# akuendig/cuda-matrix-inversion

Measured on AMD Instinct MI355X. Metric: matrix inversions/s, higher is better.
Workload: dtype f64; 1 GPU; gj64: 100000 x 64x64 fp64 Gauss-Jordan, SPD inputs (natural-order pivots verified inside the MFMA sweep; a rejected matrix is redone with partial pivoting), BASELINE configs[2]; n=64, total_batch=100000, batch_per_gpu=100000, algorithm=gj, kernel=matinv_gj_tile_f64<4, true, true>, input=SPD: R + R^T + n I

## Files before the change

### cuda-matrix-inversion_amd/csrc/tile_gj_kernels.hip

```cpp
#include "tile_impl.hpp"

namespace matinv {

template hipError_t launch_gj_tile<double>(int, BatchRef<const double>, BatchRef<double>, size_t, int *, hipStream_t);

}
```

### cuda-matrix-inversion_amd/csrc/tile_impl.hpp

```cpp
#pragma once
#include <stdio.h>
#include <stdlib.h>
#include <string.h>
#include <atomic>

#include "tile_common.hpp"
#include "tile_screen.hpp"

namespace matinv {


#define MATINV_PREP_ROW(MOV, b, a) MOV " %" #b ", %" #a "\n\t" MOV " %" #a ", 0\n\t"
#define MATINV_PREP_ZERO(MOV, a) MOV " %" #a ", 0\n\t"
#define MATINV_PREP_TAIL(MOV, save, eye) MOV " %0, %" #eye "\n\ts_nop 1\n\ts_mov_b64 exec, %" #save
#define MATINV_PREP_SAVE(save, mask) "s_and_saveexec_b64 %" #save ", %" #mask "\n\t"
template <int NT, class T>
__device__ __forceinline__ void prep_operands(typename TileGeo<T>::vec4 (&acc)[NT][NT], T (&bop)[NT], int kb, T eye)
{
    static_assert(NT >= 1 && NT <= 4, "prep_operands: one asm text per tile count");
    const int tK = kb >> 2, rK = kb & 3;
    const unsigned long long pmask = sizeof(T) == 8 ? 0x000F000F000F000FULL << (4 * rK) : 0x1111111111111111ULL << rK;
    unsigned long long save;
    auto J = [&](int i) { return (tK + i) % NT; };
    auto R = [&](int i) { return (rK + i) & 3; };
#define ROW(i) acc[tK][J(i)][rK]
#define COL(i, r) acc[J(i)][tK][R(r)]
    if constexpr (sizeof(T) == 8) {
#define MV "v_mov_b64_e32"
        if constexpr (NT == 1)
            asm volatile(MATINV_PREP_ROW(MV, 0, 1) MATINV_PREP_SAVE(5, 6)
                         MATINV_PREP_ZERO(MV, 2) MATINV_PREP_ZERO(MV, 3) MATINV_PREP_ZERO(MV, 4) MATINV_PREP_TAIL(MV, 5, 7)
                         : "=&v"(bop[J(0)]), "+v"(ROW(0)), "+v"(COL(0, 1)), "+v"(COL(0, 2)), "+v"(COL(0, 3)), "=&s"(save)
                         : "s"(pmask), "v"(eye) : "scc");
        else if constexpr (NT == 2)
            asm volatile(MATINV_PREP_ROW(MV, 0, 2) MATINV_PREP_ROW(MV, 1, 3) MATINV_PREP_SAVE(11, 12)
                         MATINV_PREP_ZERO(MV, 4) MATINV_PREP_ZERO(MV, 5) MATINV_PREP_ZERO(MV, 6)
                         MATINV_PREP_ZERO(MV, 7) MATINV_PREP_ZERO(MV, 8) MATINV_PREP_ZERO(MV, 9) MATINV_PREP_ZERO(MV, 10)
                         MATINV_PREP_TAIL(MV, 11, 13)
                         : "=&v"(bop[J(0)]), "=&v"(bop[J(1)]), "+v"(ROW(0)), "+v"(ROW(1)),
                           "+v"(COL(0, 1)), "+v"(COL(0, 2)), "+v"(COL(0, 3)),
                           "+v"(COL(1, 0)), "+v"(COL(1, 1)), "+v"(COL(1, 2)), "+v"(COL(1, 3)), "=&s"(save)
                         : "s"(pmask), "v"(eye) : "scc");
        else if constexpr (NT == 3)
            asm volatile(MATINV_PREP_ROW(MV, 0, 3) MATINV_PREP_ROW(MV, 1, 4) MATINV_PREP_ROW(MV, 2, 5) MATINV_PREP_SAVE(17, 18)
                         MATINV_PREP_ZERO(MV, 6) MATINV_PREP_ZERO(MV, 7) MATINV_PREP_ZERO(MV, 8)
                         MATINV_PREP_ZERO(MV, 9) MATINV_PREP_ZERO(MV, 10) MATINV_PREP_ZERO(MV, 11) MATINV_PREP_ZERO(MV, 12)
                         MATINV_PREP_ZERO(MV, 13) MATINV_PREP_ZERO(MV, 14) MATINV_PREP_ZERO(MV, 15) MATINV_PREP_ZERO(MV, 16)
                         MATINV_PREP_TAIL(MV, 17, 19)
                         : "=&v"(bop[J(0)]), "=&v"(bop[J(1)]), "=&v"(bop[J(2)]), "+v"(ROW(0)), "+v"(ROW(1)), "+v"(ROW(2)),
                           "+v"(COL(0, 1)), "+v"(COL(0, 2)), "+v"(COL(0, 3)),
                           "+v"(COL(1, 0)), "+v"(COL(1, 1)), "+v"(COL(1, 2)), "+v"(COL(1, 3)),
                           "+v"(COL(2, 0)), "+v"(COL(2, 1)), "+v"(COL(2, 2)), "+v"(COL(2, 3)), "=&s"(save)
                         : "s"(pmask), "v"(eye) : "scc");
        else
            asm volatile(MATINV_PREP_ROW(MV, 0, 4) MATINV_PREP_ROW(MV, 1, 5) MATINV_PREP_ROW(MV, 2, 6) MATINV_PREP_ROW(MV, 3, 7)
                         MATINV_PREP_SAVE(23, 24)
                         MATINV_PREP_ZERO(MV, 8) MATINV_PREP_ZERO(MV, 9) MATINV_PREP_ZERO(MV, 10)
                         MATINV_PREP_ZERO(MV, 11) MATINV_PREP_ZERO(MV, 12) MATINV_PREP_ZERO(MV, 13) MATINV_PREP_ZERO(MV, 14)
                         MATINV_PREP_ZERO(MV, 15) MATINV_PREP_ZERO(MV, 16) MATINV_PREP_ZERO(MV, 17) MATINV_PREP_ZERO(MV, 18)
                         MATINV_PREP_ZERO(MV, 19) MATINV_PREP_ZERO(MV, 20) MATINV_PREP_ZERO(MV, 21) MATINV_PREP_ZERO(MV, 22)
                         MATINV_PREP_TAIL(MV, 23, 25)
                         : "=&v"(bop[J(0)]), "=&v"(bop[J(1)]), "=&v"(bop[J(2)]), "=&v"(bop[J(3)]),
                           "+v"(ROW(0)), "+v"(ROW(1)), "+v"(ROW(2)), "+v"(ROW(3)),
                           "+v"(COL(0, 1)), "+v"(COL(0, 2)), "+v"(COL(0, 3)),
                           "+v"(COL(1, 0)), "+v"(COL(1, 1)), "+v"(COL(1, 2)), "+v"(COL(1, 3)),
                           "+v"(COL(2, 0)), "+v"(COL(2, 1)), "+v"(COL(2, 2)), "+v"(COL(2, 3)),
                           "+v"(COL(3, 0)), "+v"(COL(3, 1)), "+v"(COL(3, 2)), "+v"(COL(3, 3)), "=&s"(save)
                         : "s"(pmask), "v"(eye) : "scc");
#undef MV
    } else {
#define MV "v_mov_b32_e32"
        if constexpr (NT == 1)
            asm volatile(MATINV_PREP_ROW(MV, 0, 1) MATINV_PREP_SAVE(5, 6)
                         MATINV_PREP_ZERO(MV, 2) MATINV_PREP_ZERO(MV, 3) MATINV_PREP_ZERO(MV, 4) MATINV_PREP_TAIL(MV, 5, 7)
                         : "=&v"(bop[J(0)]), "+v"(ROW(0)), "+v"(COL(0, 1)), "+v"(COL(0, 2)), "+v"(COL(0, 3)), "=&s"(save)
                         : "s"(pmask), "v"(eye) : "scc");
        else if constexpr (NT == 2)
            asm volatile(MATINV_PREP_ROW(MV, 0, 2) MATINV_PREP_ROW(MV, 1, 3) MATINV_PREP_SAVE(11, 12)
                         MATINV_PREP_ZERO(MV, 4) MATINV_PREP_ZERO(MV, 5) MATINV_PREP_ZERO(MV, 6)
                         MATINV_PREP_ZERO(MV, 7) MATINV_PREP_ZERO(MV, 8) MATINV_PREP_ZERO(MV, 9) MATINV_PREP_ZERO(MV, 10)
                         MATINV_PREP_TAIL(MV, 11, 13)
                         : "=&v"(bop[J(0)]), "=&v"(bop[J(1)]), "+v"(ROW(0)), "+v"(ROW(1)),
                           "+v"(COL(0, 1)), "+v"(COL(0, 2)), "+v"(COL(0, 3)),
                           "+v"(COL(1, 0)), "+v"(COL(1, 1)), "+v"(COL(1, 2)), "+v"(COL(1, 3)), "=&s"(save)
                         : "s"(pmask), "v"(eye) : "scc");
        else if constexpr (NT == 3)
            asm volatile(MATINV_PREP_ROW(MV, 0, 3) MATINV_PREP_ROW(MV, 1, 4) MATINV_PREP_ROW(MV, 2, 5) MATINV_PREP_SAVE(17, 18)
                         MATINV_PREP_ZERO(MV, 6) MATINV_PREP_ZERO(MV, 7) MATINV_PREP_ZERO(MV, 8)
                         MATINV_PREP_ZERO(MV, 9) MATINV_PREP_ZERO(MV, 10) MATINV_PREP_ZERO(MV, 11) MATINV_PREP_ZERO(MV, 12)
                         MATINV_PREP_ZERO(MV, 13) MATINV_PREP_ZERO(MV, 14) MATINV_PREP_ZERO(MV, 15) MATINV_PREP_ZERO(MV, 16)
                         MATINV_PREP_TAIL(MV, 17, 19)
                         : "=&v"(bop[J(0)]), "=&v"(bop[J(1)]), "=&v"(bop[J(2)]), "+v"(ROW(0)), "+v"(ROW(1)), "+v"(ROW(2)),
                           "+v"(COL(0, 1)), "+v"(COL(0, 2)), "+v"(COL(0, 3)),
                           "+v"(COL(1, 0)), "+v"(COL(1, 1)), "+v"(COL(1, 2)), "+v"(COL(1, 3)),
                           "+v"(COL(2, 0)), "+v"(COL(2, 1)), "+v"(COL(2, 2)), "+v"(COL(2, 3)), "=&s"(save)
                         : "s"(pmask), "v"(eye) : "scc");
        else
            asm volatile(MATINV_PREP_ROW(MV, 0, 4) MATINV_PREP_ROW(MV, 1, 5) MATINV_PREP_ROW(MV, 2, 6) MATINV_PREP_ROW(MV, 3, 7)
                         MATINV_PREP_SAVE(23, 24)
                         MATINV_PREP_ZERO(MV, 8) MATINV_PREP_ZERO(MV, 9) MATINV_PREP_ZERO(MV, 10)
                         MATINV_PREP_ZERO(MV, 11) MATINV_PREP_ZERO(MV, 12) MATINV_PREP_ZERO(MV, 13) MATINV_PREP_ZERO(MV, 14)
                         MATINV_PREP_ZERO(MV, 15) MATINV_PREP_ZERO(MV, 16) MATINV_PREP_ZERO(MV, 17) MATINV_PREP_ZERO(MV, 18)
                         MATINV_PREP_ZERO(MV, 19) MATINV_PREP_ZERO(MV, 20) MATINV_PREP_ZERO(MV, 21) MATINV_PREP_ZERO(MV, 22)
                         MATINV_PREP_TAIL(MV, 23, 25)
                         : "=&v"(bop[J(0)]), "=&v"(bop[J(1)]), "=&v"(bop[J(2)]), "=&v"(bop[J(3)]),
                           "+v"(ROW(0)), "+v"(ROW(1)), "+v"(ROW(2)), "+v"(ROW(3)),
                           "+v"(COL(0, 1)), "+v"(COL(0, 2)), "+v"(COL(0, 3)),
                           "+v"(COL(1, 0)), "+v"(COL(1, 1)), "+v"(COL(1, 2)), "+v"(COL(1, 3)),
                           "+v"(COL(2, 0)), "+v"(COL(2, 1)), "+v"(COL(2, 2)), "+v"(COL(2, 3)),
                           "+v"(COL(3, 0)), "+v"(COL(3, 1)), "+v"(COL(3, 2)), "+v"(COL(3, 3)), "=&s"(save)
                         : "s"(pmask), "v"(eye) : "scc");
#undef MV
    }
#undef ROW
#undef COL
}
#undef MATINV_PREP_ROW
#undef MATINV_PREP_ZERO
#undef MATINV_PREP_TAIL
#undef MATINV_PREP_SAVE

template <class T, int NT, bool FULL, bool LOOKAHEAD, bool EARLY = false>
__device__ __forceinline__ void gj_tile_body(BatchRef<const T> Ain, BatchRef<T> Xout, int *info, int n_rt, unsigned batch,
                                             int *work_count, int *work_list, T *panel, const int *in_count, const int *in_list)
{
    typedef TileGeo<T> G;
    typedef typename G::vec4 vec4;
    typedef typename G::vec2 vec2;
    constexpr int N = 16 * NT;
    constexpr int NKB = 4 * NT;
    constexpr bool PAIRED = FULL && (NT % 2 == 0);
    const int l = threadIdx.x;

    const unsigned todo = in_count ? (unsigned)*in_count : batch;
    for (unsigned item = blockIdx.x; item < todo; item += gridDim.x) {
        const unsigned mat = in_list ? (unsigned)in_list[item] : item;
        const T *A = Ain.at_uniform(mat);
        T *X = Xout.at_uniform(mat);
        int n = FULL ? N : n_rt;
        if (!FULL) asm volatile("" : "+s"(n));
        int q = l >> 4, c = l & 15;
        const unsigned lane_off = (unsigned)(G::trow(0, l >> 4) * n + (l & 15));
        asm volatile("" : "+v"(q), "+v"(c));
        const T eye = G::piv(c) == q ? (T)1 : (T)0;
        vec4 acc[NT][NT];
        if (PAIRED) {
            const unsigned lane_off2 = (unsigned)(2 * G::trow(0, l >> 4) * N + 2 * (l & 15));
#pragma unroll
            for (int ti = 0; ti < NT; ++ti)
#pragma unroll
                for (int u = 0; u < NT / 2; ++u)
#pragma unroll
                    for (int r = 0; r < 4; ++r) {
                        const unsigned uoff = (unsigned)((32 * (ti >> 1) + 2 * G::trow(r, 0) + (ti & 1)) * N + 32 * u);
                        const vec2 v = __builtin_nontemporal_load(reinterpret_cast<const vec2 *>(A + uoff + lane_off2));
                        acc[ti][2 * u][r] = v[0];
                        acc[ti][2 * u + 1][r] = v[1];
                    }
        } else {
#pragma unroll
            for (int ti = 0; ti < NT; ++ti)
#pragma unroll
                for (int tj = 0; tj < NT; ++tj)
#pragma unroll
                    for (int r = 0; r < 4; ++r) {
                        const int row = 16 * ti + G::trow(r, q), col = 16 * tj + c;
                        const unsigned uoff = (unsigned)((16 * ti + G::trow(r, 0)) * n + 16 * tj);
                        const bool edge = !FULL && (ti == NT - 1 || tj == NT - 1);
                        acc[ti][tj][r] = (!edge || (row < n && col < n)) ? A[uoff + lane_off] : ((row == col) ? (T)1 : (T)0);
                    }
        }
        unsigned long long bad = 0;
        T aop[NT], bop[NT];

#ifdef MATINV_TILE_LDST_ONLY
        if (false) {
#else
        if (LOOKAHEAD) {
#endif
            panel_to_lds<NT, T>(panel, acc, 0, q, c);
            wave_lds_sync();
            panel_solve<NT>(panel, 0, q, c, aop, bad);
#pragma unroll
            for (int kb = 0; kb < NKB; ++kb) {
                if (!FULL && kb > 4 * (NT - 1) && kb - 4 * (NT - 1) >= G::real_blocks(n - 16 * (NT - 1))) continue;
                prep_operands<NT, T>(acc, bop, kb, eye);
                if (kb + 1 < NKB) {
                    const int tn = (kb + 1) >> 2;
#pragma unroll
                    for (int ti = 0; ti < NT; ++ti)
                        acc[ti][tn] = G::mfma(aop[ti], bop[tn], acc[ti][tn]);
                    constexpr int NB = NT * (NT - 1);
                    int pend = 0;
                    auto issue_b = [&](int count) {
#pragma unroll
                        for (int z = 0; z < count; ++z) {
                            if (pend < NB) {
                                const int tjx = pend / NT, ti = pend % NT;
                                const int tj = tjx + (tjx >= tn ? 1 : 0);
                                acc[ti][tj] = G::mfma(aop[ti], bop[tj], acc[ti][tj]);
                                ++pend;
                            }
                        }
                        __builtin_amdgcn_sched_barrier(0);
                    };
                    __builtin_amdgcn_sched_barrier(0);
                    issue_b(2);
                    wave_lds_sync();
                    panel_to_lds<NT, T>(panel, acc, kb + 1, q, c);
                    wave_lds_sync();
                    __builtin_amdgcn_sched_barrier(0);
                    T aop_next[NT];
                    PanelSolve<NT, false, T> ps;
                    constexpr int NS = PanelSolve<NT, false, T>::NSTAGE;
#pragma unroll
                    for (int s = 0; s < NS; ++s) {
                        issue_b(((NB - 2) * (s + 1)) / NS - ((NB - 2) * s) / NS);
                        ps.stage(s, panel, kb + 1, q, c, aop_next, bad);
                        __builtin_amdgcn_sched_barrier(0);
                    }
                    issue_b(NB);
#pragma unroll
                    for (int ti = 0; ti < NT; ++ti) aop[ti] = aop_next[ti];
                    if (EARLY && NT > 1 && kb == 3 && bad != 0) break;
                } else {
#pragma unroll
                    for (int ti = 0; ti < NT; ++ti)
#pragma unroll
                        for (int tj = 0; tj < NT; ++tj)
                            acc[ti][tj] = G::mfma(aop[ti], bop[tj], acc[ti][tj]);
                }
            }
        } else {
#ifdef MATINV_TILE_LDST_ONLY
            (void)aop, (void)bop;
#else
#pragma unroll
            for (int kb = 0; kb < NKB; ++kb) {
                if (!FULL && kb > 4 * (NT - 1) && kb - 4 * (NT - 1) >= G::real_blocks(n - 16 * (NT - 1))) continue;
                panel_to_lds<NT, T>(panel, acc, kb, q, c);
                wave_lds_sync();
                panel_solve<NT>(panel, kb, q, c, aop, bad);
                wave_lds_sync();
                prep_operands<NT, T>(acc, bop, kb, eye);
#pragma unroll
                for (int ti = 0; ti < NT; ++ti)
#pragma unroll
                    for (int tj = 0; tj < NT; ++tj)
                        acc[ti][tj] = G::mfma(aop[ti], bop[tj], acc[ti][tj]);
            }
#endif
        }

        if (bad == 0) {
            if (PAIRED) {
                const unsigned lane_off2 = (unsigned)(2 * G::trow(0, l >> 4) * N + 2 * (l & 15));
#pragma unroll
                for (int ti = 0; ti < NT; ++ti)
#pragma unroll
                    for (int u = 0; u < NT / 2; ++u)
#pragma unroll
                        for (int r = 0; r < 4; ++r) {
                            const unsigned uoff = (unsigned)((32 * (ti >> 1) + 2 * G::trow(r, 0) + (ti & 1)) * N + 32 * u);
                            vec2 v;
                            v[0] = acc[ti][2 * u][r];
                            v[1] = acc[ti][2 * u + 1][r];
                            __builtin_nontemporal_store(v, reinterpret_cast<vec2 *>(X + uoff + lane_off2));
                        }
            } else {
#pragma unroll
                for (int ti = 0; ti < NT; ++ti)
#pragma unroll
                    for (int tj = 0; tj < NT; ++tj)
#pragma unroll
                        for (int r = 0; r < 4; ++r) {
                            const int row = 16 * ti + G::trow(r, q), col = 16 * tj + c;
                            const unsigned uoff = (unsigned)((16 * ti + G::trow(r, 0)) * n + 16 * tj);
                            const bool edge = !FULL && (ti == NT - 1 || tj == NT - 1);
                            if (!edge || (row < n && col < n)) X[uoff + lane_off] = acc[ti][tj][r];
                        }
            }
            if (info && l == 0) info[mat] = 0;
        } else if (l == 0) {
            const int slot = atomicAdd(work_count, 1);
            work_list[slot] = (int)mat;
        }
        if (LOOKAHEAD) wave_lds_sync();
    }
}


template <int NT, bool FULL, bool LOOKAHEAD, bool EARLY = false>
__global__ __launch_bounds__(64, 2) void matinv_gj_tile_f64(BatchRef<const double> Ain,
                                                                                 BatchRef<double> Xout, int *info,
                                                                                 int n_rt, unsigned batch,
                                                                                 int *work_count, int *work_list, const int *in_count,
                                                                                 const int *in_list)
{
    __shared__ __attribute__((aligned(16))) double panel[16 * NT * 4];
    gj_tile_body<double, NT, FULL, LOOKAHEAD, EARLY>(Ain, Xout, info, n_rt, batch, work_count, work_list, panel, in_count, in_list);
}

template <int NT, bool FULL, bool LOOKAHEAD, bool EARLY = false>
__global__ __launch_bounds__(64, FULL ? 4 : 3) void matinv_gj_tile_f32(BatchRef<const float> Ain, BatchRef<float> Xout, int *info,
                                                           int n_rt, unsigned batch, int *work_count, int *work_list, const int *in_count,
                                                           const int *in_list)
{
    __shared__ __attribute__((aligned(16))) float panel[16 * NT * 4];
    gj_tile_body<float, NT, FULL, LOOKAHEAD, EARLY>(Ain, Xout, info, n_rt, batch, work_count, work_list, panel, in_count, in_list);
}

template <class T>
struct SpdGp {
    const T *a, *c, *d, *e;
    T *out;
};

template <class T, int NT, bool FULL, bool GP = false>
__device__ __forceinline__ void spd_tile_body(BatchRef<const T> Ain, BatchRef<T> Xout, int *info, int n_rt, unsigned batch,
                                              int *work_count, int *work_list, T *panel, SpdGp<T> gp = SpdGp<T>())
{
    typedef TileGeo<T> G;
    typedef typename G::vec4 vec4;
    constexpr int N = 16 * NT;
    constexpr int NKB = 4 * NT;
    constexpr int TSTRIDE = 17;
    const int l = threadIdx.x;

    for (unsigned mat = blockIdx.x; mat < batch; mat += gridDim.x) {
        const T *A = Ain.at_uniform(mat);
        T *X = Xout.at_uniform(mat);
        int n = FULL ? N : n_rt;
        if (!FULL) asm volatile("" : "+s"(n));
        int q = l >> 4, c = l & 15;
        const unsigned lane_off = (unsigned)((l >> 4) * n + (l & 15));
        asm volatile("" : "+v"(q), "+v"(c));

        vec4 acc[NT][NT];
#pragma unroll
        for (int ti = 0; ti < NT; ++ti)
#pragma unroll
            for (int tj = 0; tj < NT; ++tj) {
                if (tj > ti) continue;
#pragma unroll
                for (int r = 0; r < 4; ++r) {
                    const int row = 16 * ti + G::trow(r, q), col = 16 * tj + c;
                    T v;
                    if (ti == tj) {
                        const int hi = row > col ? row : col, lo = row > col ? col : row;
                        v = (FULL || ti < NT - 1 || (row < n && col < n)) ? A[(unsigned)(lo * n + hi)] : ((row == col) ? (T)1 : (T)0);
                        if (GP && row == col && (FULL || ti < NT - 1 || row < n)) v += gp.c[(size_t)mat * n + row];
                    } else {
                        v = (FULL || ti < NT - 1 || (row < n && col < n)) ? A[(unsigned)(col * n + row)] : (T)0;
                    }
                    acc[ti][tj][r] = v;
                }
            }
        (void)lane_off;
        unsigned long long bad = 0;
        T aop[NT], bop[NT];

        spd_panel_to_lds<NT, T>(panel, acc, 0, q, c);
        wave_lds_sync();
        {
            PanelSolve<NT, true, T> ps0;
#pragma unroll
            for (int s = 0; s < PanelSolve<NT, true, T>::NSTAGE; ++s) ps0.stage(s, panel, 0, q, c, aop, bop, bad);
        }
#pragma unroll
        for (int kb = 0; kb < NKB; ++kb) {
            const int tK = kb >> 2;
            if (!FULL && kb > 4 * (NT - 1) && kb - 4 * (NT - 1) >= G::real_blocks(n - 16 * (NT - 1))) continue;
            spd_prep_operands<NT, T>(acc, bop, kb, q, c);
            if (kb + 1 < NKB) {
                const int tn = (kb + 1) >> 2;
#pragma unroll
                for (int ti = 0; ti < NT; ++ti) {
                    if (ti < tn) continue;
                    acc[ti][tn] = G::mfma(aop[ti], bop[tn], acc[ti][tn]);
                }
#pragma unroll
                for (int tj = 0; tj < NT; ++tj) {
                    if (tj >= tn) continue;
                    acc[tn][tj] = G::mfma(aop[tn], bop[tj], acc[tn][tj]);
                }
                constexpr int NB = NT * (NT + 1) / 2 - NT;
                constexpr int NS = PanelSolve<NT, true, T>::NSTAGE;
                T aop_next[NT], bop_next[NT];
                PanelSolve<NT, true, T> ps;
                int count = 0, ev = 0;
                auto run_events = [&](bool flush) {
#pragma unroll
                    for (int e = 0; e < NS + 1; ++e) {
                        const int lead = NB < 2 ? NB : 2;
                        const int thr = (e == 0) ? lead : lead + ((NB - lead) * e) / NS;
                        if (e == ev && (flush || thr <= count)) {
                            __builtin_amdgcn_sched_barrier(0);
                            if (e == 0) {
                                wave_lds_sync();
                                spd_panel_to_lds<NT, T>(panel, acc, kb + 1, q, c);
                                wave_lds_sync();
                            } else {
                                ps.stage(e - 1, panel, kb + 1, q, c, aop_next, bop_next, bad);
                            }
                            __builtin_amdgcn_sched_barrier(0);
                            ++ev;
                        }
                    }
                };
                run_events(false);
#pragma unroll
                for (int ti = 0; ti < NT; ++ti)
#pragma unroll
                    for (int tj = 0; tj < NT; ++tj) {
                        if (tj > ti || ti == tn || tj == tn) continue;
                        acc[ti][tj] = G::mfma(aop[ti], bop[tj], acc[ti][tj]);
                        ++count;
                        run_events(false);
                    }
                run_events(true);
#pragma unroll
                for (int ti = 0; ti < NT; ++ti) { aop[ti] = aop_next[ti]; bop[ti] = bop_next[ti]; }
            } else {
#pragma unroll
                for (int ti = 0; ti < NT; ++ti)
#pragma unroll
                    for (int tj = 0; tj < NT; ++tj) {
                        if (tj > ti) continue;
                        acc[ti][tj] = G::mfma(aop[ti], bop[tj], acc[ti][tj]);
                    }
            }
            (void)tK;
        }

        if (GP && bad == 0) {
            const T *va = gp.a + (size_t)mat * n;
            const T *vd = gp.d ? gp.d + (size_t)mat * n : va;
            wave_lds_sync();
            T *const sa = panel, *const sd = panel + N;
#pragma unroll
            for (int k = 0; k < (N + 63) / 64; ++k) {
                const int i = l + 64 * k;
                if (i < N) {
                    sa[i] = (FULL || i < n) ? va[i] : (T)0;
                    sd[i] = (FULL || i < n) ? vd[i] : (T)0;
                }
            }
            wave_lds_sync();
            T s = 0;
#pragma unroll
            for (int tj = 0; tj < NT; ++tj) {
                const T ac = sa[16 * tj + c], dc = sd[16 * tj + c];
#pragma unroll
                for (int ti = tj; ti < NT; ++ti)
#pragma unroll
                    for (int r = 0; r < 4; ++r) {
                        const int row = 16 * ti + G::trow(r, q);
                        const T ar = sa[row], dr = sd[row];
                        const T wgt = (ti == tj) ? ar * dc : fma_t(ar, dc, dr * ac);
                        s = fma_t(acc[ti][tj][r], wgt, s);
                    }
            }
#pragma unroll
            for (int off = 32; off >= 1; off >>= 1) s += __shfl_xor(s, off);
            if (l == 0) {
                gp.out[mat] = gp.d ? -s : gp.e[mat] + s;
                if (info) info[mat] = 0;
            }
        } else if (bad == 0) {
#pragma unroll
            for (int ti = 0; ti < NT; ++ti)
#pragma unroll
                for (int tj = 0; tj < NT; ++tj) {
                    if (tj > ti) continue;
#pragma unroll
                    for (int r = 0; r < 4; ++r) {
                        const int row = 16 * ti + G::trow(r, q), col = 16 * tj + c;
                        if (FULL || ti < NT - 1 || (row < n && col < n)) X[(unsigned)(row * n + col)] = -acc[ti][tj][r];
                    }
                    if (tj < ti) {
                        wave_lds_sync();
#pragma unroll
                        for (int r = 0; r < 4; ++r) panel[G::trow(r, q) * TSTRIDE + c] = -acc[ti][tj][r];
                        wave_lds_sync();
#pragma unroll
                        for (int r = 0; r < 4; ++r) {
                            const int row = 16 * tj + G::trow(r, q), col = 16 * ti + c;
                            const T v = panel[c * TSTRIDE + G::trow(r, q)];
                            if (FULL || ti < NT - 1 || (row < n && col < n)) X[(unsigned)(row * n + col)] = v;
                        }
                    }
                }
            if (info && l == 0) info[mat] = 0;
        } else if (l == 0) {
            const int slot = atomicAdd(work_count, 1);
            work_list[slot] = (int)mat;
        }
        wave_lds_sync();
    }
}


template <int NT, bool FULL>
__global__ __launch_bounds__(64, NT >= 7 ? 1 : (NT >= 5 ? 2 : (NT >= 4 ? 3 : 4))) void matinv_spd_tile_f64(BatchRef<const double> Ain, BatchRef<double> Xout,
                                                                          int *info, int n_rt, unsigned batch,
                                                                          int *work_count, int *work_list)
{
    __shared__ __attribute__((aligned(16))) double panel[(16 * NT * 4 > 16 * 17) ? 16 * NT * 4 : 16 * 17];
    spd_tile_body<double, NT, FULL>(Ain, Xout, info, n_rt, batch, work_count, work_list, panel);
}

template <int NT, bool FULL>
#ifndef MATINV_SPD_WIDE_OCC
#define MATINV_SPD_WIDE_OCC 2
#endif
__global__ __launch_bounds__(64, NT >= 9 ? MATINV_SPD_WIDE_OCC : (NT >= 7 ? 2 : (NT >= 5 ? 3 : 4))) void matinv_spd_tile_f32(BatchRef<const float> Ain, BatchRef<float> Xout, int *info,
                                                            int n_rt, unsigned batch, int *work_count, int *work_list)
{
    __shared__ __attribute__((aligned(16))) float panel[(16 * NT * 4 > 16 * 17) ? 16 * NT * 4 : 16 * 17];
    spd_tile_body<float, NT, FULL>(Ain, Xout, info, n_rt, batch, work_count, work_list, panel);
}

template <int NT>
__global__ __launch_bounds__(64, NT >= 7 ? 1 : 2) void matinv_gp_spd_tile_f64(const double *As, const double *Bs, const double *Cs, const double *Ds,
                                                               const double *Es, double *out, int *info, int n_rt, unsigned batch,
                                                               int *work_count, int *work_list)
{
    __shared__ __attribute__((aligned(16))) double panel[(16 * NT * 4 > 16 * 17) ? 16 * NT * 4 : 16 * 17];
    BatchRef<const double> A{Bs, (size_t)n_rt * n_rt, nullptr};
    BatchRef<double> X{nullptr, 0, nullptr};
    spd_tile_body<double, NT, false, true>(A, X, info, n_rt, batch, work_count, work_list, panel, SpdGp<double>{As, Cs, Ds, Es, out});
}
template <int NT>
__global__ __launch_bounds__(64, NT >= 9 ? MATINV_SPD_WIDE_OCC : 2) void matinv_gp_spd_tile_f32(const float *As, const float *Bs, const float *Cs, const float *Ds,
                                                               const float *Es, float *out, int *info, int n_rt, unsigned batch,
                                                               int *work_count, int *work_list)
{
    __shared__ __attribute__((aligned(16))) float panel[(16 * NT * 4 > 16 * 17) ? 16 * NT * 4 : 16 * 17];
    BatchRef<const float> A{Bs, (size_t)n_rt * n_rt, nullptr};
    BatchRef<float> X{nullptr, 0, nullptr};
    spd_tile_body<float, NT, false, true>(A, X, info, n_rt, batch, work_count, work_list, panel, SpdGp<float>{As, Cs, Ds, Es, out});
}


bool tile_policy_use_screen(bool f64, int nt);
template <class T>
hipError_t launch_gj_tile_natural(int n, BatchRef<const T> A, BatchRef<T> X, size_t batch, int *info, hipStream_t stream)
{
    constexpr bool F64 = sizeof(T) == 8;
    const TileShape s = tile_shape(n);
    const bool rowlane2 = rowlane2_natural_use(F64, n);
    const bool screen = !rowlane2 && tile_policy_use_screen(F64, s.nt);
    return with_scratch_ints((screen ? 3 : 2) * batch + 4, 4, stream, [&](int *ws) {
        int *const rej_count = ws, *const sing_count = ws + 1, *const acc_count = ws + 2;
        int *const rej_list = ws + 4, *const sing_list = ws + 4 + batch, *const acc_list = ws + 4 + 2 * batch;
        hipError_t e;
        if (rowlane2) {
            e = enqueue_gj_rowlane2<T>(n, A, X, batch, info, stream, rej_count, rej_list);
        } else {
            const unsigned grid = tile_grid(batch, F64 ? 8u : 16u), b = (unsigned)batch;
            const unsigned sgrid = tile_grid(batch, 16u, 1u);
            with_tile<1, 4>(s, [&](auto NT, auto FULL) {
                constexpr bool EARLY = NT >= 3;
                if constexpr (F64) {
                    if (!screen) {
                        hipLaunchKernelGGL((matinv_gj_tile_f64<NT, FULL, true>), dim3(grid), dim3(64), 0, stream, A, X, info, n, b, rej_count,
                                           rej_list, nullptr, nullptr);
                        return;
                    }
                    hipLaunchKernelGGL((matinv_gj_tile_screen_f64<NT, FULL>), dim3(sgrid), dim3(64), 0, stream, A, n, b, rej_count, rej_list,
                                       acc_count, acc_list);
                    hipLaunchKernelGGL((matinv_gj_tile_f64<NT, FULL, true, EARLY>), dim3(grid), dim3(64), 0, stream, A, X, info, n, b, rej_count,
                                       rej_list, acc_count, acc_list);
                } else {
                    if (!screen) {
                        hipLaunchKernelGGL((matinv_gj_tile_f32<NT, FULL, true>), dim3(grid), dim3(64), 0, stream, A, X, info, n, b, rej_count,
                                           rej_list, nullptr, nullptr);
                        return;
                    }
                    hipLaunchKernelGGL((matinv_gj_tile_screen_f32<NT, FULL>), dim3(sgrid), dim3(64), 0, stream, A, n, b, rej_count, rej_list,
                                       acc_count, acc_list);
                    hipLaunchKernelGGL((matinv_gj_tile_f32<NT, FULL, true, EARLY>), dim3(grid), dim3(64), 0, stream, A, X, info, n, b, rej_count,
                                       rej_list, acc_count, acc_list);
                }
            });
            e = hipGetLastError();
        }
        if (e == hipSuccess)
            e = launch_gj_tilep_worklist<T>(n, A, X, batch, rej_count, rej_list, sing_count, sing_list, info, stream,
                                            tile_policy_record(F64, s.nt, batch), screen);
        return e;
    });
}

template <class T>
hipError_t launch_gj_tile(int n, BatchRef<const T> A, BatchRef<T> X, size_t batch, int *info, hipStream_t stream)
{
    if (!tile_family_supports<T>(n)) return hipErrorInvalidValue;
    if (batch == 0) return hipSuccess;
    if (n > 64) return launch_gj_tile4<T>(n, A, X, batch, info, stream);
    if (tile_policy_use_pivot(sizeof(T) == 8, tile_shape(n).nt)) return launch_gj_tilep<T>(n, A, X, batch, info, stream);
    return launch_gj_tile_natural<T>(n, A, X, batch, info, stream);
}

constexpr TileShape spd_tile_shape(bool f64, int n) { return {(n + 15) / 16, n % 16 == 0 && (f64 || n < 128)}; }

hipError_t enqueue_spd_tile_big_f32(int n, BatchRef<const float> A, BatchRef<float> X, unsigned grid, unsigned b, int *info, int *ws,
                                    hipStream_t stream);
template <class T>
hipError_t launch_gp_spd_tile(int n, const T *As, const T *Bs, const T *Cs, const T *Ds, const T *Es, T *out, size_t batch, int *info,
                              hipStream_t stream)
{
    if (!gp_spd_tile_supports(sizeof(T) == 8, n)) return hipErrorInvalidValue;
    if (batch == 0) return hipSuccess;
    return with_scratch_ints(batch + 1, 1, stream, [&](int *ws) {
        const unsigned grid = tile_grid(batch, 8u), b = (unsigned)batch;
        hipError_t e = hipSuccess;
        if constexpr (sizeof(T) == 8) {
            if (n <= 96) hipLaunchKernelGGL((matinv_gp_spd_tile_f64<6>), dim3(grid), dim3(64), 0, stream, As, Bs, Cs, Ds, Es, out, info, n, b, ws, ws + 1);
            else e = enqueue_gp_spd_tile_wide_f64(n, As, Bs, Cs, Ds, Es, out, grid, b, info, ws, stream);
        } else {
            if (n <= 112) hipLaunchKernelGGL((matinv_gp_spd_tile_f32<7>), dim3(grid), dim3(64), 0, stream, As, Bs, Cs, Ds, Es, out, info, n, b, ws, ws + 1);
            else if (n <= 128) hipLaunchKernelGGL((matinv_gp_spd_tile_f32<8>), dim3(grid), dim3(64), 0, stream, As, Bs, Cs, Ds, Es, out, info, n, b, ws, ws + 1);
            else e = enqueue_gp_spd_tile_wide_f32(n, As, Bs, Cs, Ds, Es, out, grid, b, info, ws, stream);
        }
        if (e == hipSuccess) e = hipGetLastError();
        if (e == hipSuccess) e = launch_gp_lds_worklist<T>(n, As, Bs, Cs, Ds, Es, out, ws, ws + 1, info, stream);
        return e;
    });
}

}
```

Baseline: 69.00 million inversions/s.

## Interleave final-step MFMA updates with output stores in f64 64x64 tile kernel

For the 64x64 fp64 lookahead kernel, the last elimination step now computes column-pair tiles one at a time and stores each finished pair immediately, instead of doing all MFMAs and then all stores. Input loads are regrouped by column pair with scheduling barriers. The aim is to overlap global store latency with the remaining matrix-core work at the end of each matrix. Stores are now issued before the pivot check completes for later tiles only when no bad pivot was seen. Optional timestamp instrumentation is added behind a compile flag.

```diff
diff --git a/cuda-matrix-inversion_amd/csrc/tile_gj_kernels.hip b/cuda-matrix-inversion_amd/csrc/tile_gj_kernels.hip
--- a/cuda-matrix-inversion_amd/csrc/tile_gj_kernels.hip
+++ b/cuda-matrix-inversion_amd/csrc/tile_gj_kernels.hip
@@ -5,3 +5,11 @@
 template hipError_t launch_gj_tile<double>(int, BatchRef<const double>, BatchRef<double>, size_t, int *, hipStream_t);
 
 }
+
+#ifdef MATINV_TILE_STAMPS
+extern "C" int matinv_debug_tile_stamps(unsigned long long *dst, size_t rows)
+{
+    if (rows > matinv::TILE_STAMP_ROWS) return -1;
+    return (int)hipMemcpyFromSymbol(dst, HIP_SYMBOL(matinv::g_tile_stamps), rows * matinv::TILE_STAMP_WORDS * sizeof(unsigned long long));
+}
+#endif
diff --git a/cuda-matrix-inversion_amd/csrc/tile_impl.hpp b/cuda-matrix-inversion_amd/csrc/tile_impl.hpp
--- a/cuda-matrix-inversion_amd/csrc/tile_impl.hpp
+++ b/cuda-matrix-inversion_amd/csrc/tile_impl.hpp
@@ -120,6 +120,22 @@
 #undef MATINV_PREP_TAIL
 #undef MATINV_PREP_SAVE
 
+#ifdef MATINV_TILE_STAMPS
+constexpr unsigned TILE_STAMP_ROWS = 1u << 17, TILE_STAMP_WORDS = 8;
+static __device__ unsigned long long g_tile_stamps[TILE_STAMP_ROWS * TILE_STAMP_WORDS];
+__device__ __forceinline__ unsigned long long tile_stamp()
+{
+    unsigned long long t;
+    __builtin_amdgcn_sched_barrier(0);
+    asm volatile("s_memtime %0\n\ts_waitcnt lgkmcnt(0)" : "=s"(t) : : "memory");
+    __builtin_amdgcn_sched_barrier(0);
+    return t;
+}
+#define MATINV_STAMP(i) if constexpr (SPLIT) stamp[i] = tile_stamp()
+#else
+#define MATINV_STAMP(i)
+#endif
+
 template <class T, int NT, bool FULL, bool LOOKAHEAD, bool EARLY = false>
 __device__ __forceinline__ void gj_tile_body(BatchRef<const T> Ain, BatchRef<T> Xout, int *info, int n_rt, unsigned batch,
                                              int *work_count, int *work_list, T *panel, const int *in_count, const int *in_list)
@@ -130,6 +146,12 @@
     constexpr int N = 16 * NT;
     constexpr int NKB = 4 * NT;
     constexpr bool PAIRED = FULL && (NT % 2 == 0);
+    constexpr bool SPLIT = PAIRED && LOOKAHEAD && !EARLY && NT == 4 && sizeof(T) == 8;
+#ifdef MATINV_TILE_LDST_ONLY
+    constexpr bool SWEEP_STORES = false;
+#else
+    constexpr bool SWEEP_STORES = SPLIT;
+#endif
     const int l = threadIdx.x;
 
     const unsigned todo = in_count ? (unsigned)*in_count : batch;
@@ -144,19 +166,26 @@
         asm volatile("" : "+v"(q), "+v"(c));
         const T eye = G::piv(c) == q ? (T)1 : (T)0;
         vec4 acc[NT][NT];
+#ifdef MATINV_TILE_STAMPS
+        unsigned long long stamp[8] = {};
+#endif
+        MATINV_STAMP(0);
         if (PAIRED) {
             const unsigned lane_off2 = (unsigned)(2 * G::trow(0, l >> 4) * N + 2 * (l & 15));
 #pragma unroll
-            for (int ti = 0; ti < NT; ++ti)
-#pragma unroll
-                for (int u = 0; u < NT / 2; ++u)
+            for (int o = 0; o < (SPLIT ? NT / 2 : NT); ++o) {
+#pragma unroll
+                for (int i = 0; i < (SPLIT ? NT : NT / 2); ++i)
 #pragma unroll
                     for (int r = 0; r < 4; ++r) {
+                        const int ti = SPLIT ? i : o, u = SPLIT ? o : i;
                         const unsigned uoff = (unsigned)((32 * (ti >> 1) + 2 * G::trow(r, 0) + (ti & 1)) * N + 32 * u);
                         const vec2 v = __builtin_nontemporal_load(reinterpret_cast<const vec2 *>(A + uoff + lane_off2));
                         acc[ti][2 * u][r] = v[0];
                         acc[ti][2 * u + 1][r] = v[1];
                     }
+                if (SPLIT) __builtin_amdgcn_sched_barrier(0);
+            }
         } else {
 #pragma unroll
             for (int ti = 0; ti < NT; ++ti)
@@ -172,6 +201,17 @@
         }
         unsigned long long bad = 0;
         T aop[NT], bop[NT];
+        auto store_pair = [&](int ti, int u) {
+            const unsigned lane_off2 = (unsigned)(2 * G::trow(0, l >> 4) * N + 2 * (l & 15));
+#pragma unroll
+            for (int r = 0; r < 4; ++r) {
+                const unsigned uoff = (unsigned)((32 * (ti >> 1) + 2 * G::trow(r, 0) + (ti & 1)) * N + 32 * u);
+                vec2 v;
+                v[0] = acc[ti][2 * u][r];
+                v[1] = acc[ti][2 * u + 1][r];
+                __builtin_nontemporal_store(v, reinterpret_cast<vec2 *>(X + uoff + lane_off2));
+            }
+        };
 
 #ifdef MATINV_TILE_LDST_ONLY
         if (false) {
@@ -180,6 +220,12 @@
 #endif
             panel_to_lds<NT, T>(panel, acc, 0, q, c);
             wave_lds_sync();
+            MATINV_STAMP(1);
+#ifdef MATINV_TILE_STAMPS
+            MATINV_STAMP(2);
+            asm volatile("s_waitcnt vmcnt(0)" ::: "memory");
+            MATINV_STAMP(3);
+#endif
             panel_solve<NT>(panel, 0, q, c, aop, bad);
 #pragma unroll
             for (int kb = 0; kb < NKB; ++kb) {
@@ -223,6 +269,21 @@
 #pragma unroll
                     for (int ti = 0; ti < NT; ++ti) aop[ti] = aop_next[ti];
                     if (EARLY && NT > 1 && kb == 3 && bad != 0) break;
+                } else if constexpr (SWEEP_STORES) {
+                    MATINV_STAMP(4);
+                    if (bad == 0) {
+#pragma unroll
+                        for (int p = 0; p <= 2 * NT; ++p) {
+                            if (p < 2 * NT) {
+                                const int u = p / NT, ti = p % NT;
+                                acc[ti][2 * u] = G::mfma(aop[ti], bop[2 * u], acc[ti][2 * u]);
+                                acc[ti][2 * u + 1] = G::mfma(aop[ti], bop[2 * u + 1], acc[ti][2 * u + 1]);
+                            }
+                            if (p > 0) store_pair((p - 1) % NT, (p - 1) / NT);
+                            __builtin_amdgcn_sched_barrier(0);
+                        }
+                    }
+                    MATINV_STAMP(5);
                 } else {
 #pragma unroll
                     for (int ti = 0; ti < NT; ++ti)
@@ -253,20 +314,12 @@
         }
 
         if (bad == 0) {
-            if (PAIRED) {
-                const unsigned lane_off2 = (unsigned)(2 * G::trow(0, l >> 4) * N + 2 * (l & 15));
+            if (SWEEP_STORES) {
+            } else if (PAIRED) {
 #pragma unroll
                 for (int ti = 0; ti < NT; ++ti)
 #pragma unroll
-                    for (int u = 0; u < NT / 2; ++u)
-#pragma unroll
-                        for (int r = 0; r < 4; ++r) {
-                            const unsigned uoff = (unsigned)((32 * (ti >> 1) + 2 * G::trow(r, 0) + (ti & 1)) * N + 32 * u);
-                            vec2 v;
-                            v[0] = acc[ti][2 * u][r];
-                            v[1] = acc[ti][2 * u + 1][r];
-                            __builtin_nontemporal_store(v, reinterpret_cast<vec2 *>(X + uoff + lane_off2));
-                        }
+                    for (int u = 0; u < NT / 2; ++u) store_pair(ti, u);
             } else {
 #pragma unroll
                 for (int ti = 0; ti < NT; ++ti)
@@ -285,9 +338,22 @@
             const int slot = atomicAdd(work_count, 1);
             work_list[slot] = (int)mat;
         }
+#ifdef MATINV_TILE_STAMPS
+        if constexpr (SPLIT) {
+            asm volatile("s_waitcnt vmcnt(0)" ::: "memory");
+            MATINV_STAMP(6);
+            unsigned hw, xcc;
+            asm volatile("s_getreg_b32 %0, hwreg(HW_REG_HW_ID)\n\ts_getreg_b32 %1, hwreg(HW_REG_XCC_ID)" : "=s"(hw), "=s"(xcc));
+            stamp[7] = hw | (unsigned long long)xcc << 32;
+            if (l == 0 && mat < TILE_STAMP_ROWS)
+#pragma unroll
+                for (int i = 0; i < 8; ++i) g_tile_stamps[(size_t)mat * TILE_STAMP_WORDS + i] = stamp[i];
+        }
+#endif
         if (LOOKAHEAD) wave_lds_sync();
     }
 }
+#undef MATINV_STAMP
 
 
 template <int NT, bool FULL, bool LOOKAHEAD, bool EARLY = false>
```

Result: no change. 69.06 million inversions/s (median of 6 runs) (+0.1%).
